# ariana-spalter/human-robot-gym

Hardware: AMD Instinct MI355X
Metric: env steps/sec (whole node), ReachHuman+shield 4096 envs (higher is better)
Workload: dtype f64

## Files before the change

human-robot-gym_amd/csrc/hrgym_device.h:

```cpp
#pragma once
#include <hip/hip_runtime.h>
#include <stdint.h>

#include "../../include/hrgym.h"
#include "../../include/hrgym_state.h"

#define NV HRG_NV
#define NARM HRG_NARM
#ifndef HRG_BOX
#define HRG_BOX 0
#endif
#ifndef HRG_LIFT
#define HRG_LIFT 0
#endif
#ifndef HRG_HANDOVER
#define HRG_HANDOVER 0
#endif
#ifndef HRG_STACK
#define HRG_STACK 0
#endif
#ifndef HRG_HULLS
#define HRG_HULLS 0
#endif
#ifndef HRG_HAMMER
// ... 126 lines not shown
  int32_t hb_maxdepth;
  double sol_K, sol_Bd;
  double rcap_hl[HRG_NRCAP], hcap_hl[HRG_NHB];
  int32_t hb_njump;
  int32_t hb_jump[4][HRG_NHB];
  int32_t phase_mask;
  hrg_path brake_full;
  double brake_T, brake_ds;
  int32_t hc_n;
  struct alignas(32) HcRec { double th, v, al; int32_t kj, pad; } hc[HRG_NHCAP_MAX];
  int32_t n_self;
  struct alignas(8) SelfPair { int32_t i, j; } self_ij[64];
  int32_t n_chk;
  int32_t chk_i[32], chk_j[32];
  hrg_clip_table clips;
  const double* pose_tab;
  const double* hull_dev;
  double hull_cen[HRG_NHULL][3];
  unsigned long long* mpr_fallback;
  double fric_D[NV + 1], fric_lim[NV + 1];
  double eul_hd[NV], eul_rhd[2];
  int32_t eul_fingers, eul_pad;
  double rcap_mid[HRG_NRCAP][3];
};

struct Contact {
  int32_t g1, g2, b1, b2;
  double dist, n[3], pos[3];
};

#define ROW_CON0 24
#define ROW_WELD0 (ROW_CON0 + 4 * NCON_DYN)
#if HRG_HAMMER
#define HROW_NFRIC 8
#define HROW_LIM0 9
#define HROW_NLIM 25
#define HROW_EQ0 27
#define HROW_CON0 36
#define HROW_NEQ 9
#define NROW 128
#elif HRG_STACK
#define SROW_WELD0 24
#define SROW_CON0 36
#define NROW HRG_NROW_STACK
#elif HRG_BOX && (HRG_HANDOVER || HRG_LIFT)
#define NROW (ROW_WELD0 + 6)
// ... 480 lines not shown
    if (g > 0) lo = w; else hi = w;
    const double sd = d1 >= 0 ? 1.0 : -1.0;
    const double T1p = sd * (fabs(d1) >= vtri ? 1.0 / amax : (fabs(d1) > 0 ? 1.0 / fsqrt(jmax * fabs(d1)) : 0.0));
    const double T2p = w >= vtri ? 1.0 / amax : (w > 0 ? 1.0 / fsqrt(jmax * w) : 0.0);
    const double dncp = 0.5 * T1 + 0.5 * (vm + w) * T1p + 0.5 * T2 + 0.5 * w * T2p;
    const double gp = T1p + T2p - dncp / w - rest / (w * w);
    double nw = gp < 0 ? w - g / gp : 0.5 * (lo + hi);
    if (!(nw > lo && nw < hi)) nw = 0.5 * (lo + hi);
    const double step = fabs(nw - w);
    w = nw;
    found = true;
    if (step <= 4e-16 * (1.0 + w) || hi - lo <= 4e-16 * (1.0 + hi)) break;
  }
  if (!found || !(w > 0)) return;
  const double tc = (Dm - dist_nocruise(vm, w, amax, jmax)) / w;
  if (!(tc >= 0)) return;
  int n = tl.n0;
  scurve(tl.v, tl.sg * w, amax, jmax, dur + n, jerk + n);
  n += 3;
  dur[n] = tc; jerk[n] = 0; n++;
  scurve(tl.sg * w, 0, amax, jmax, dur + n, jerk + n);
}

DI void ltt_eval(const hrg_ltt* L, int j, double s, double* q, double* v, double* a) {
  double qq = L->q0[j], vv = L->v0[j], aa = L->a0[j], t = s;
  if (t < 0) t = 0;
  for (int i = 0; i < HRG_LTT_NSEG; i++) {
    double d = L->dur[j][i], jj = L->jerk[j][i];
    if (t < d) {
      *q = qq + vv * t + 0.5 * aa * t * t + jj * t * t * t * SIXTH;
      *v = vv + aa * t + 0.5 * jj * t * t;
      *a = aa + jj * t;
      return;
    }
    qq += vv * d + 0.5 * aa * d * d + jj * d * d * d * SIXTH;
    vv += aa * d + 0.5 * jj * d * d;
    aa += jj * d;
    t -= d;
  }
  *q = L->qT[j]; *v = 0; *a = 0;
}

DI void ltt_eval2(const hrg_ltt* L, int j, double sa, double sb, double* qa, double* va, double* aa_, double* qb) {
  double qq = L->q0[j], vv = L->v0[j], aa = L->a0[j], ta = sa < 0 ? 0 : sa, tb = sb < 0 ? 0 : sb;
  bool done_a = false;
  for (int i = 0; i < HRG_LTT_NSEG; i++) {
    const double d = L->dur[j][i], jj = L->jerk[j][i];
    if (!done_a && ta < d) {
      *qa = qq + vv * ta + 0.5 * aa * ta * ta + jj * ta * ta * ta * SIXTH;
      *va = vv + aa * ta + 0.5 * jj * ta * ta;
      *aa_ = aa + jj * ta;
      done_a = true;
    }
    if (tb < d) {
      *qb = qq + vv * tb + 0.5 * aa * tb * tb + jj * tb * tb * tb * SIXTH;
      return;
    }
    qq += vv * d + 0.5 * aa * d * d + jj * d * d * d * SIXTH;
    vv += aa * d + 0.5 * jj * d * d;
    aa += jj * d;
    ta -= d;
    tb -= d;
  }
  if (!done_a) { *qa = L->qT[j]; *va = 0; *aa_ = 0; }
  *qb = L->qT[j];
}

__host__ DI void path_plan(hrg_path* P, double s0, double v0, double a0, double ve, double amax, double jmax) {
  P->s0 = s0; P->v0 = v0; P->a0 = a0; P->k = 0;
  for (int i = 0; i < 3; i++) { P->dur[i] = 0; P->jerk[i] = 0; }
  if (fabs(v0 - ve) < 1e-12 && fabs(a0) < 1e-12) { P->v0 = ve; P->a0 = 0; return; }
  double v_at = v0 + a0 * fabs(a0) / (2 * jmax);
  double dir = ve >= v_at ? 1.0 : -1.0;
  double A = dir * a0, dv = dir * (ve - v0);
  double apk = amax > A ? amax : A;
  double t1 = (apk - A) / jmax, t3 = apk / jmax;
  double dv2 = dv - 0.5 * (A + apk) * t1 - 0.5 * apk * t3, t2;
  if (dv2 >= 0) t2 = dv2 / apk;
  else {
    double r = 0.5 * A * A + jmax * dv;
    apk = sqrt(r > 0 ? r : 0);
    if (apk < A) apk = A;
    t1 = (apk - A) / jmax; t2 = 0; t3 = apk / jmax;
  }
  P->dur[0] = t1; P->dur[1] = t2; P->dur[2] = t3;
  P->jerk[0] = dir * jmax; P->jerk[1] = 0; P->jerk[2] = -dir * jmax;
}
__host__ DI double path_total(const hrg_path* P) { return P->dur[0] + P->dur[1] + P->dur[2]; }
// ... 220 lines not shown
```

human-robot-gym_amd/csrc/hrgym_hip.hip:

```cpp
#include <hip/hip_runtime.h>

#include <algorithm>
#include <cmath>
#include <cstdio>
#include <cstring>
#include <cstdlib>
#include <initializer_list>
#include <limits>
#include <memory>
#include <string>
#include <vector>

#include "hrgym_kernels.h"

template <class MD>
DI void impedance(const MD& m, double x0, double* imp) {
  const double d0 = m.solimp[0], dmax = m.solimp[1], width = m.solimp[2], mid = m.solimp[3], power = m.solimp[4];
  const double x = fabs(x0) / width;
  double y;
  if (x >= 1) y = 1;
  else if (x <= 0) y = 0;
  else if (x <= mid) { const double u = x / mid; y = u * u * mid; }
  else { const double u = (1 - x) / (1 - mid); y = 1 - u * u * (1 - mid); }
  (void)power;
// ... 2358 lines not shown
    eef_update(dm_);
    s.low_level_time = s.low_level_time + 1;
  }
  wave_sync();
  STAMP_FLUSH(lane);
  return crash | busy_out;
}

DI int env_step(const DevModel* __restrict__ dm_, int lane, int e, int64_t own_gid, double* __restrict__ action, float* obs, float* term_obs,
                 float* reward, uint8_t* done, int32_t* info, double* dbg_r, double* dbg_h, int32_t* dbg_nh, int32_t* fair) {
  const ModelPtr dm = uniform_model(dm_);
  Lds& L = g_L;
  const auto& m = dm->m;
  hrg_env_state& s = L.st;
  (void)fair;
  const int64_t gid = s.stream_id;
  int has_collision = 0, collision_type = HRG_COL_NULL, crash = 0;
  STAMP_INIT(lane);
  if (lane < NV) L.act[lane] = lane < HRG_ACT_DIM ? action[lane] : 0.0;
  wave_sync();
#if HRG_POSE_TABLE
  human_yaw_update();
#endif
  if (m.ik_enabled) ik_action(dm_, lane);
  if (m.cp_enabled) screen_action(dm_, lane, gid);
#if HRG_LIFT
  if (m.task == HRG_TASK_LIFTING) { wave_sync(); if (lane == 0) L.act[NARM] = 1.0; wave_sync(); }
#endif
#if HRG_HAMMER
  if (!m.gripper_controllable) { wave_sync(); if (lane == 0) L.act[NARM] = 1.0; wave_sync(); }
#endif
  if ((m.cp_enabled || m.ik_enabled) && lane < HRG_ACT_DIM) action[lane] = L.act[lane];
  s.timestep = s.timestep + 1;
  L.acc_has_collision = 0; L.acc_collision_type = HRG_COL_NULL; L.acc_failsafe = 0;
  wave_sync();
  int busy = 0;
#pragma unroll 1
  for (int cyc = 0; cyc < m.n_cycles && !crash; cyc++) { const int r = cycle_body(dm_, lane, e, gid, cyc, busy, dbg_r, dbg_h, dbg_nh, fair); crash = r & 1; busy = r >> 1; }
#if HRG_FAIR
  fair_publish(fair, lane, -1);
  __builtin_amdgcn_s_setprio(0);
#endif
  has_collision = L.acc_has_collision; collision_type = L.acc_collision_type;
  double goal[NARM];
  for (int j = 0; j < NARM; j++) goal[j] = s.cur_goal[j];
#if HRG_BOX
// ... 601 lines not shown
  }
  if (lane < NV) { st[HRG_MC_EUL_HD + lane] = dm_->eul_hd[lane]; re[HRG_MC_EUL_HD + lane] = c.eul_hd; }
  if (lane < 2) { st[HRG_MC_EUL_RHD + lane] = dm_->eul_rhd[lane]; re[HRG_MC_EUL_RHD + lane] = c.eul_rhd; }
  if (lane == 0) { st[HRG_MC_EUL_FINGERS] = dm_->eul_fingers; re[HRG_MC_EUL_FINGERS] = c.eul_fingers; }
  if (lane < 3 * HRG_NRCAP) { st[HRG_MC_RCAP_MID + lane] = (&dm_->rcap_mid[0][0])[lane]; re[HRG_MC_RCAP_MID + lane] = c.rcap_mid; }
}
#endif

__global__ __launch_bounds__(64) void HRG_SYM(hrg_chain_fk_kernel)(const DevModel* __restrict__ dm_, const double* __restrict__ q, int n, int shield_on, double* __restrict__ out) {
  const int lane = hrg_lane(), k = (int)blockIdx.x;
  if (k >= n) return;
  Lds& L = g_L;
  const double* qk = q + (size_t)k * 3 * NARM;
  if (lane < NARM) { L.cq[lane] = qk[lane]; L.qe[lane] = qk[NARM + lane]; }
  if (lane < NV) L.st.qpos[lane] = lane < NARM ? qk[2 * NARM + lane] : 0.0;
  wave_sync();
  robot_chain_fk(dm_, lane, shield_on != 0);
  double* o = out + (size_t)k * HRG_CFK_DIM;
  for (int j = lane; j < 9 * NV; j += 64) o[HRG_CFK_KR + j] = (&L.kR[0][0])[j];
  if (lane < 3 * NV) o[HRG_CFK_KP + lane] = (&L.kp[0][0])[lane];
  for (int j = lane; j < 2 * HRG_NSHIELD_RCAP * 6; j += 64) o[HRG_CFK_SCAP + j] = shield_on ? (&L.scap[0][0][0])[j] : 0.0;
}

#define HRG_NP_HAS_BOX (HRG_BOX || HRG_STACK || HRG_HAMMER)
#define HRG_NP_HAS_BB (HRG_STACK || HRG_HAMMER || HRG_LIFT)
#define HRG_NP_BOX_LANES 32
#define HRG_NP_BB_LANES (HRG_STACK ? 6 : HRG_HAMMER ? 4 : 1)
__global__ __launch_bounds__(64) void HRG_SYM(hrg_narrowphase_kernel)(int kind, const double* __restrict__ qs, int n, double* __restrict__ out) {
  const int lane = hrg_lane(), per = kind == HRG_NP_SEGSEG ? 64 : kind == HRG_NP_BOXBOX ? HRG_NP_BB_LANES : HRG_NP_BOX_LANES, k = (int)blockIdx.x * per + lane;
  const bool on = lane < per && k < n;
  const double* q = qs + (size_t)(on ? k : 0) * HRG_NP_QDIM;
  double* o = out + (size_t)(on ? k : 0) * HRG_NP_ODIM;
  if (on) for (int a = 0; a < HRG_NP_ODIM; a++) o[a] = 0.0;
  if (kind == HRG_NP_SEGSEG) {
    if (on) {
      double c1[3], c2[3];
      o[0] = seg_seg(q, q + 3, q + 6, q + 9, c1, c2);
      for (int a = 0; a < 3; a++) { o[1 + a] = c1[a]; o[4 + a] = c2[a]; }
    }
    return;
  }
#if HRG_NP_HAS_BOX || HRG_NP_HAS_BB
  Lds& L = g_L;
  double* W = &L.Jc[0][0];
  const int sl = on ? lane : 0;
#endif
// ... 53 lines not shown
    return;
  }
#endif
}

typedef void hrg_launch_step_fn(int n_envs, hipStream_t st, const DevModel* dm, hrg_env_state* states, double* actions, float* obs, float* term_obs, float* reward, uint8_t* done,
                                int32_t* info, double* dbg_r, double* dbg_h, int32_t* dbg_nh, int64_t env_id0, float* scratch_obs, void* objs, StepOrder ord);
typedef void hrg_launch_reset_fn(int n_envs, hipStream_t st, const DevModel* dm, hrg_env_state* states, const uint8_t* mask, float* obs, int64_t env_id0, void* objs);
extern "C" __attribute__((visibility("hidden"))) hrg_launch_step_fn HRG_SYM(hrg_launch_step);
extern "C" __attribute__((visibility("hidden"))) hrg_launch_reset_fn HRG_SYM(hrg_launch_reset);
extern "C" void HRG_SYM(hrg_launch_step)(int n_envs, hipStream_t st, const DevModel* dm, hrg_env_state* states, double* actions, float* obs, float* term_obs, float* reward, uint8_t* done,
                                         int32_t* info, double* dbg_r, double* dbg_h, int32_t* dbg_nh, int64_t env_id0, float* scratch_obs, void* objs, StepOrder ord) {
  hipLaunchKernelGGL(HRG_SYM(hrg_step_kernel), HRG_LAUNCH_DIMS(n_envs), 0, st, dm, states, actions, obs, term_obs, reward, done, info, dbg_r, dbg_h, dbg_nh, env_id0, scratch_obs, (ObjState*)objs,
                     n_envs, ord);
}
extern "C" void HRG_SYM(hrg_launch_reset)(int n_envs, hipStream_t st, const DevModel* dm, hrg_env_state* states, const uint8_t* mask, float* obs, int64_t env_id0, void* objs) {
  hipLaunchKernelGGL(HRG_SYM(hrg_reset_kernel), HRG_LAUNCH_DIMS(n_envs), 0, st, dm, states, mask, obs, env_id0, (ObjState*)objs, n_envs);
}
typedef void hrg_launch_chain_fk_fn(int n, const DevModel* dm, const double* q, int shield_on, double* out);
extern "C" __attribute__((visibility("hidden"))) hrg_launch_chain_fk_fn HRG_SYM(hrg_launch_chain_fk);
extern "C" void HRG_SYM(hrg_launch_chain_fk)(int n, const DevModel* dm, const double* q, int shield_on, double* out) {
  hipLaunchKernelGGL(HRG_SYM(hrg_chain_fk_kernel), dim3((unsigned)n), dim3(64), 0, 0, dm, q, n, shield_on, out);
}
typedef int hrg_launch_narrowphase_fn(int kind, int n, const double* q, double* out);
extern "C" __attribute__((visibility("hidden"))) hrg_launch_narrowphase_fn HRG_SYM(hrg_launch_narrowphase);
extern "C" int HRG_SYM(hrg_launch_narrowphase)(int kind, int n, const double* q, double* out) {
  const bool has = kind == HRG_NP_SEGSEG || (HRG_NP_HAS_BOX && (kind == HRG_NP_SEGBOX || kind == HRG_NP_CAPBOX)) || (HRG_NP_HAS_BB && kind == HRG_NP_BOXBOX);
  if (!has) return 0;
  const int per = kind == HRG_NP_SEGSEG ? 64 : kind == HRG_NP_BOXBOX ? HRG_NP_BB_LANES : HRG_NP_BOX_LANES;
  hipLaunchKernelGGL(HRG_SYM(hrg_narrowphase_kernel), dim3((unsigned)((n + per - 1) / per)), dim3(64), 0, 0, kind, q, n, out);
  return 1;
}

#ifdef HRG_STAMPS
#if HRG_BASE_TU
extern "C" int hrg_debug_stamps_slow(double* out, unsigned long long thresh, int reset) {
  unsigned long long h[34];
  if (hipMemcpyFromSymbol(h, HIP_SYMBOL(g_stamps_slow), sizeof h) != hipSuccess) return -1;
  for (int i = 0; i < 34; i++) out[i] = (double)h[i];
  if (reset) { memset(h, 0, sizeof h); hipMemcpyToSymbol(HIP_SYMBOL(g_stamps_slow), h, sizeof h); }
  hipMemcpyToSymbol(HIP_SYMBOL(g_slow_thresh), &thresh, sizeof thresh);
  return 0;
}
#endif
extern "C" int HRG_SYM(hrg_debug_stamps)(double* out, int reset) {
  unsigned long long h[32];
// ... 27 lines not shown
```

human-robot-gym_amd/csrc/hrgym_host_batch.h:

```cpp

struct TaskTraits;
struct hrg_batch {
  int device = 0;
  int32_t n_envs = 0;
  int64_t env_id0 = 0;
  DeviceMem mem;
  DevModel* d_model = nullptr;
  double* d_frames = nullptr;
  double* d_pose = nullptr;
  size_t pose_bytes = 0;
  double* d_hull = nullptr;
  bool hulls = false;
  unsigned long long* d_mpr_fallback = nullptr;
  hrg_env_state* d_states = nullptr;
  double* d_rcaps = nullptr;
  double* d_hcaps = nullptr;
  int32_t* d_nh = nullptr;
  float* d_scratch_obs = nullptr;
  hrg_box_state* d_boxes = nullptr;
  hrg_stack_state* d_stacks = nullptr;
  hrg_hammer_state* d_hammers = nullptr;
  int32_t* d_order = nullptr;
  int32_t parity = 0;
  const TaskTraits* traits = nullptr;
  bool ik = false;
  bool has_expert = false;
  hrg_expert_desc expert;
  ExpertBuffers ex;
  std::unique_ptr<DeviceMem> ex_mem;
  bool has_dataset = false;
  hrg_dataset_desc dataset;
  DatasetDev ds;
  std::unique_ptr<DeviceMem> ds_mem;
// ... 11 lines not shown
  static int32_t* tab[64] = {nullptr};
  if (device < 0 || device >= 64) return nullptr;
  if (!tab[device]) {
    int32_t* p = nullptr;
    if (hipMalloc(&p, sizeof(int32_t) * HRG_FAIR_SLOTS) != hipSuccess) return nullptr;
    if (hipMemset(p, 0, sizeof(int32_t) * HRG_FAIR_SLOTS) != hipSuccess) { hipFree(p); return nullptr; }
    tab[device] = p;
  }
  return tab[device];
}

enum { HRG_FAM_REACH, HRG_FAM_BOX, HRG_FAM_HO, HRG_FAM_LIFT, HRG_FAM_STACK, HRG_FAM_HAMMER, HRG_NFAMILY };
#define HRG_VARIANTS(X)                                              \
  X(HRG_FAM_REACH, 0, )          X(HRG_FAM_REACH, 1, _hull)          \
  X(HRG_FAM_BOX, 0, _box)        X(HRG_FAM_BOX, 1, _box_hull)        \
  X(HRG_FAM_HO, 0, _ho)          X(HRG_FAM_HO, 1, _ho_hull)          \
  X(HRG_FAM_LIFT, 0, _lift)      X(HRG_FAM_LIFT, 1, _lift_hull)      \
  X(HRG_FAM_STACK, 0, _stack)    X(HRG_FAM_STACK, 1, _stack_hull)    \
  X(HRG_FAM_HAMMER, 0, _hammer)  X(HRG_FAM_HAMMER, 1, _hammer_hull)
#define X(family, hulls, sfx)                                                                  \
  extern "C" __attribute__((visibility("hidden"))) hrg_launch_step_fn hrg_launch_step##sfx;    \
  extern "C" __attribute__((visibility("hidden"))) hrg_launch_reset_fn hrg_launch_reset##sfx;  \
  extern "C" __attribute__((visibility("hidden"))) hrg_launch_chain_fk_fn hrg_launch_chain_fk##sfx;  \
  extern "C" __attribute__((visibility("hidden"))) hrg_launch_narrowphase_fn hrg_launch_narrowphase##sfx;
HRG_VARIANTS(X)
#undef X
struct Variant { hrg_launch_step_fn* step; hrg_launch_reset_fn* reset; hrg_launch_chain_fk_fn* chain_fk; hrg_launch_narrowphase_fn* narrowphase; };
struct VariantTable { Variant v[HRG_NFAMILY][2]; };
static constexpr VariantTable make_variants() {
  VariantTable t{};
#define X(family, hulls, sfx) t.v[family][hulls] = Variant{hrg_launch_step##sfx, hrg_launch_reset##sfx, hrg_launch_chain_fk##sfx, hrg_launch_narrowphase##sfx};
  HRG_VARIANTS(X)
#undef X
  return t;
}
static const VariantTable g_variants = make_variants();

enum { HRG_OBJ_NONE, HRG_OBJ_BOXES, HRG_OBJ_STACKS, HRG_OBJ_HAMMERS };
struct TaskTraits {
  int task, family, objs;
  bool pose_table;
  bool dataset;
  unsigned experts, sirs;
};
#define E(x) (1u << HRG_EXPERT_##x)
#define S(x) (1u << HRG_SIR_##x)
static constexpr TaskTraits HRG_TASKS[] = {
  {HRG_TASK_REACH, HRG_FAM_REACH, HRG_OBJ_NONE, true, true, E(REACH), S(REACH)},
  {HRG_TASK_PICK_PLACE, HRG_FAM_BOX, HRG_OBJ_BOXES, false, true, E(PICK_PLACE), S(PICK_PLACE)},
  {HRG_TASK_INSPECTION, HRG_FAM_BOX, HRG_OBJ_BOXES, false, true, 0, 0},
  {HRG_TASK_POINTING, HRG_FAM_BOX, HRG_OBJ_BOXES, false, true, 0, 0},
  {HRG_TASK_HANDOVER_H2R, HRG_FAM_HO, HRG_OBJ_BOXES, false, true, E(PICK_PLACE), S(PICK_PLACE)},
  {HRG_TASK_HANDOVER_R2H, HRG_FAM_HO, HRG_OBJ_BOXES, false, true, E(PICK_PLACE), S(PICK_PLACE)},
  {HRG_TASK_LIFTING, HRG_FAM_LIFT, HRG_OBJ_BOXES, true, true, E(LIFTING), S(LIFTING)},
// ... 184 lines not shown
    double se, ve, ae;
    path_plan(&hm->brake_full, 0.0, 1.0, 0.0, desc->failsafe_sdot, desc->path_amax, desc->path_jmax);
    hm->brake_T = path_total(&hm->brake_full);
    path_eval(&hm->brake_full, hm->brake_T, desc->failsafe_sdot, &se, &ve, &ae);
    hm->brake_ds = se;
  }
#ifdef HRG_STAMPS
  if (const char* pm = getenv("HRG_PHASE_MASK")) hm->phase_mask = atoi(pm);
#endif
  hm->clips = *clips;
  if (desc->robot_hulls) hull_centroids(desc->hull_verts, desc->hull_off, hm->hull_cen);
}

static int batch_upload(hrg_batch* b, const hrg_model_desc* desc, const hrg_clip_table* clips, DevModel* hm) {
  DeviceMem& m = b->mem;
  const size_t frames = (size_t)clips->total_frames;
  bool ok = m.upload(b->d_frames, clips->frames, HRG_FRAME_DIM * frames);
  if (ok && b->traits->pose_table) {
    b->pose_bytes = sizeof(double) * HRG_POSE_DIM * frames;
    ok = m.zeros(b->d_pose, HRG_POSE_DIM * frames);
  }
  if (ok && desc->robot_hulls)
    ok = m.upload(b->d_hull, desc->hull_verts, 3 * (size_t)desc->hull_off[HRG_NHULL]) && m.zeros(b->d_mpr_fallback, 1);
  hm->clips.frames = b->d_frames;
  hm->pose_tab = b->d_pose;
  hm->hull_dev = b->d_hull;
  hm->mpr_fallback = b->d_mpr_fallback;
  if (!ok || !m.upload(b->d_model, hm, 1)) return nomem("batch", m);
  hipLaunchKernelGGL(hrg_model_constants_kernel, dim3(1), dim3(64), 0, 0, b->d_model);
  HIPCHK(hipGetLastError());
  HIPCHK(hipDeviceSynchronize());
  if (b->d_pose) {
    hipLaunchKernelGGL(hrg_pose_table_kernel, dim3((unsigned)clips->total_frames), dim3(64), 0, 0, b->d_model, b->d_pose);
    HIPCHK(hipGetLastError());
    HIPCHK(hipDeviceSynchronize());
  }
  return HRG_OK;
}

static int batch_env_arrays(hrg_batch* b) {
  const size_t n = (size_t)b->n_envs;
  std::vector<hrg_env_state> init(n);
  memset(init.data(), 0, sizeof(hrg_env_state) * n);
  for (auto& s : init) s.episode = -1;
  std::vector<int32_t> ord(2 * n + 4, 0);
  for (size_t e = 0; e < n; e++) ord[e] = ord[n + e] = (int32_t)e;
  DeviceMem& m = b->mem;
// ... 369 lines not shown
  }), "hrg_debug_cull_box");
}

int hrg_debug_model_constants(hrg_batch* b, double* out_host) {
  if (!b || !out_host) return fail(HRG_ERR_INVALID, "null argument");
  HIPCHK(hipSetDevice(b->device));
  return tap_result(hrg_run_tap(nullptr, 0, out_host, sizeof(double) * 2 * HRG_MC_DIM, [&](void** d) {
    hipMemset(d[0], 0, sizeof(double) * 2 * HRG_MC_DIM);
    hipLaunchKernelGGL(hrg_model_constants_tap_kernel, dim3(1), dim3(64), 0, 0, b->d_model, 0.0, (double*)d[0]);
  }), "hrg_debug_model_constants");
}

int hrg_debug_chain_fk(hrg_batch* b, const double* q_host, int32_t n, int32_t shield_on, double* out_host) {
  if (!b || !q_host || !out_host || n < 1 || n > 64) return fail(HRG_ERR_INVALID, "null argument or n outside 1..64");
  HIPCHK(hipSetDevice(b->device));
  void* objs;
  const Variant& v = batch_variant(b, &objs);
  const TapBuf in[] = {{q_host, sizeof(double) * 3 * NARM * (size_t)n}};
  return tap_result(hrg_run_tap(in, 1, out_host, sizeof(double) * HRG_CFK_DIM * (size_t)n, [&](void** d) {
    v.chain_fk((int)n, b->d_model, (const double*)d[0], shield_on ? 1 : 0, (double*)d[1]);
  }), "hrg_debug_chain_fk");
}

int hrg_debug_narrowphase(hrg_batch* b, int32_t kind, const double* queries_host, int32_t n, double* out_host) {
  if (!b || !queries_host || !out_host || n < 1 || n > HRG_NP_MAX) return fail(HRG_ERR_INVALID, "null argument or n outside 1..HRG_NP_MAX");
  if (kind < HRG_NP_SEGSEG || kind > HRG_NP_BOXBOX) return fail(HRG_ERR_INVALID, "no such kind of narrowphase query");
  HIPCHK(hipSetDevice(b->device));
  void* objs;
  const Variant& v = batch_variant(b, &objs);
  bool has = true;
  const TapBuf in[] = {{queries_host, sizeof(double) * HRG_NP_QDIM * (size_t)n}};
  const bool ok = hrg_run_tap(in, 1, out_host, sizeof(double) * HRG_NP_ODIM * (size_t)n, [&](void** d) {
    has = v.narrowphase((int)kind, (int)n, (const double*)d[0], (double*)d[1]) != 0;
  });
  if (!has) return fail(HRG_ERR_UNSUPPORTED, "this batch's kernel variant does not compile that routine");
  return tap_result(ok, "hrg_debug_narrowphase");
}

}
```

human-robot-gym_amd/csrc/hrgym_kernels.h:

```cpp
#pragma once
#include "hrgym_device.h"
#if HRG_HULLS
#include "hrgym_hull.h"
#endif

DI double chain_dot(double a0, double a1, double a2, double b0, double b1, double b2) {
#pragma clang fp contract(off)
  return __builtin_fma(a2, b2, __builtin_fma(a0, b0, a1 * b1));
}
DI double chain_acc(double a0, double a1, double a2, double b0, double b1, double b2) {
  return __builtin_fma(a2, b2, __builtin_fma(a1, b1, __builtin_fma(a0, b0, 0.0)));
}
DI void robot_chain_fk(const DevModel* __restrict__ dm_, int lane, bool shield_on) {
  const ModelPtr dm = uniform_model(dm_);
  Lds& L = g_L;
  if (lane < 3 * NARM && (lane >= 2 * NARM || shield_on)) {
    const int cfg = lane / NARM, i = lane - NARM * cfg;
    const double q = cfg == 0 ? L.cq[i] : (cfg == 1 ? L.qe[i] : L.st.qpos[i]);
    double sn, cs;
    sincos_small(q, &sn, &cs);
    LdsF64* o = lds_lane_base(&L.rc[0][0] + 2 * lane);
    o[0] = sn; o[1] = cs;
  }
  wave_sync();
// ... 496 lines not shown
    clip = clip_of(dm, gid, s.episode, anim_index);
  }
  s.anim_index = anim_index; s.anim_start_time = anim_start; s.animation_time = at;
#if HRG_BOX
  human_pose_fk(dm_, lane, clip, at, hold_body, hold_left);
#else
  human_pose_fk(dm_, lane, clip, at);
#endif
}

PH_SHIELD void shield_step(const DevModel* __restrict__ dm_, int lane, int e, double* __restrict__ dbg_r, double* __restrict__ dbg_h, int32_t* __restrict__ dbg_nh) {
  const ModelPtr dm = uniform_model(dm_);
  Lds& L = g_L;
  const auto& m = dm->m;
  hrg_env_state& s = L.st;
  const double dt = m.timestep, t = s.time;
  const bool shield_on = m.shield_type != HRG_SHIELD_OFF;
  const bool have_vel = s.n_meas >= 1 && t > s.meas_prev_t;
  if (lane < NARM) { L.cq[lane] = s.des_q[lane]; L.cv[lane] = s.des_v[lane]; L.ca[lane] = s.des_a[lane]; }
  wave_sync();
  int use_cand = 0;
  if (s.new_goal) {
    double nq = 0, nv = 0, na = 0;
    if (lane < NARM) ltt_eval(&s.ltt, lane, s.path_s, &nq, &nv, &na);
    const bool bad = lane < NARM && fabs(na) > m.a_max_ltt[lane];
    if (!__any(bad)) {
      use_cand = 1;
      double tj = 0;
      LttTail tail;
      tail.n0 = 0; tail.v = tail.sg = tail.Dm = tail.vm = tail.w = 0;
      if (lane < NARM) {
        ltt_plan_joint(&L.cand, lane, nq, nv, na, s.new_goal_q[lane], m.v_max_ltt[lane], m.a_max_ltt[lane], m.j_max_ltt[lane], &tail);
        for (int i = 0; i < HRG_LTT_NSEG; i++) tj += L.cand.dur[lane][i];
      }
      const double Tall = wave_max(tj);
      L.cand.T = Tall;
      if (m.ltt_time_sync && lane < NARM) ltt_sync_joint(&L.cand, lane, Tall, m.a_max_ltt[lane], m.j_max_ltt[lane], tail);
    }
    wave_sync();
  }
  STAMP(10);
  const hrg_ltt* Lp = use_cand ? &L.cand : &s.ltt;
  const double ps = use_cand ? 0.0 : s.path_s, pv = s.path_v, pa = s.path_a;
  hrg_path fs2;
  double s1, v1, a1, se, Tb;
  const bool pfl = m.shield_type == HRG_SHIELD_PFL, steady = pv == 1.0 && pa == 0.0;
  if (steady) { s1 = ps + dt; v1 = 1.0; a1 = 0.0; }
  else {
    hrg_path rec;
    path_plan(&rec, ps, pv, pa, 1.0, m.path_amax, m.path_jmax);
    path_eval(&rec, dt, 1.0, &s1, &v1, &a1);
  }
  double ve_fs = m.failsafe_sdot;
  if (pfl) {
    double q_, d1_ = 0, d2_;
    if (lane < NARM) ltt_eval(Lp, lane, s1, &q_, &d1_, &d2_);
    const double vc = wave_sum(lane < NARM ? fabs(d1_) * m.pfl_reach[lane] : 0.0);
    ve_fs = vc > m.pfl_v_safe ? m.pfl_v_safe / vc : 1.0;
  }
  if (steady && !pfl) {
    fs2.s0 = s1; fs2.v0 = 1.0; fs2.a0 = 0.0; fs2.k = 0.0;
    for (int a = 0; a < 3; a++) { fs2.dur[a] = dm->brake_full.dur[a]; fs2.jerk[a] = dm->brake_full.jerk[a]; }
    Tb = dm->brake_T;
    se = s1 + dm->brake_ds;
  } else {
    double ve_, ae;
    path_plan(&fs2, s1, v1, a1, ve_fs, m.path_amax, m.path_jmax);
    Tb = path_total(&fs2);
    path_eval(&fs2, Tb, ve_fs, &se, &ve_, &ae);
  }
  s1 = uniform_f64(s1); v1 = uniform_f64(v1); a1 = uniform_f64(a1); se = uniform_f64(se); Tb = uniform_f64(Tb);
  fs2.s0 = uniform_f64(fs2.s0); fs2.v0 = uniform_f64(fs2.v0); fs2.a0 = uniform_f64(fs2.a0); fs2.k = uniform_f64(fs2.k);
  for (int a = 0; a < 3; a++) { fs2.dur[a] = uniform_f64(fs2.dur[a]); fs2.jerk[a] = uniform_f64(fs2.jerk[a]); }
  STAMP(11);
  if (shield_on && lane < NARM) {
    double qn, q1, q2, qv;
    ltt_eval2(Lp, lane, s1, se, &qn, &q1, &q2, &qv);
    L.qe[lane] = qv;
    s.des_q[lane] = qn; s.des_v[lane] = q1 * v1; s.des_a[lane] = q1 * a1 + q2 * v1 * v1;
  }
  wave_sync();
  STAMP(12);
  robot_chain_fk(dm_, lane, shield_on);
  STAMP(13);
  int safe = 1;
  if (shield_on) {
    const double sdiff = se - ps;
    double rc_hl = 0;
    if (lane < HRG_NSHIELD_RCAP) {
      const int c = lane;
      double d[3], l1, l2;
      v3sub(d, &L.scap[0][c][0], &L.scap[1][c][0]); l1 = v3norm(d);
      v3sub(d, &L.scap[0][c][3], &L.scap[1][c][3]); l2 = v3norm(d);
      for (int a = 0; a < 6; a++) L.rc[c][a] = 0.5 * (L.scap[0][c][a] + L.scap[1][c][a]);
      L.rc[c][6] = m.scap_r[c] + m.secure_radius + 0.5 * (l1 > l2 ? l1 : l2) + m.scap_alpha[c] * sdiff * sdiff / 8.0;
      double hv[3];
      for (int a = 0; a < 3; a++) hv[a] = 0.5 * (L.rc[c][3 + a] - L.rc[c][a]);
      rc_hl = fsqrt(v3dot(hv, hv));
      L.scap[0][c][0] = rc_hl;
      if (dbg_r) for (int a = 0; a < 7; a++) dbg_r[((size_t)e * HRG_NSHIELD_RCAP + c) * 7 + a] = L.rc[c][a];
// ... 67 lines not shown
            const double reach = L.scap[0][c][0] + hl + rr + 1e-9;
            close = !(v3dot(dc, dc) > reach * reach);
          }
          if (!__any(close)) continue;
          if (close) { double x1[3], x2[3]; if (seg_seg(&L.rc[c][0], &L.rc[c][3], c1, c2, x1, x2) < rr * rr) hit = true; }
          if (__any(hit)) break;
        }
      }
      all_hit = __any(hit);
    }
    safe = !all_hit;
  }
  wave_sync();
  STAMP(14);
  for (int k = lane; k < HRG_NHJ * 3; k += 64) (&s.meas_prev[0][0])[k] = (&s.human_site[0][0])[k];
  s.meas_prev_t = t;
  if (s.n_meas < 2) s.n_meas = s.n_meas + 1;
  if (safe) {
    if (use_cand) {
      double* dst = (double*)&s.ltt;
      const double* src = (const double*)&L.cand;
      for (int k = lane; k < (int)(sizeof(hrg_ltt) / sizeof(double)); k += 64) dst[k] = src[k];
      s.new_goal = 0;
    }
    s.path_s = s1; s.path_v = v1; s.path_a = a1;
    s.safe_path = fs2;
  } else {
    const double k = s.safe_path.k + 1.0;
    s.safe_path.k = k;
    double ns, nv, na;
    const hrg_path spc = s.safe_path;
    const double vend = pfl ? path_vend(&spc) : m.failsafe_sdot;
    path_eval(&s.safe_path, k * dt, vend, &ns, &nv, &na);
    if (use_cand && s.path_v <= vend + 1e-9 && fabs(s.path_a) <= 1e-9) {
      const double adv = ns - s.path_s;
      double* dst = (double*)&s.ltt;
      const double* src = (const double*)&L.cand;
      for (int q = lane; q < (int)(sizeof(hrg_ltt) / sizeof(double)); q += 64) dst[q] = src[q];
      s.new_goal = 0;
      ns = adv;
      hrg_path sp;
      path_plan(&sp, ns, nv, na, vend, m.path_amax, m.path_jmax);
      s.safe_path = sp;
    }
    s.path_s = ns; s.path_v = nv; s.path_a = na;
  }
  s.is_safe = safe;
  wave_sync();
  if (lane < NARM && !(shield_on && safe)) {
    double qq, q1, q2;
    ltt_eval(&s.ltt, lane, s.path_s, &qq, &q1, &q2);
    s.des_q[lane] = qq; s.des_v[lane] = q1 * s.path_v; s.des_a[lane] = q1 * s.path_a + q2 * s.path_v * s.path_v;
  }
  wave_sync();
  STAMP(15);
}

DI void shield_reset(const DevModel* __restrict__ , int lane) {
  Lds& L = g_L;
  hrg_env_state& s = L.st;
  if (lane < NARM) {
    const double q = s.qpos[lane];
    s.ltt.q0[lane] = q; s.ltt.qT[lane] = q;
    s.des_q[lane] = q; s.new_goal_q[lane] = q; s.goal_qpos[lane] = q;
  }
  s.is_safe = 1;
}

#if HRG_STACK || HRG_HAMMER || HRG_LIFT
#define BB_TIE 1e-9
#define BB_ON (1 + 1e-12)
struct BBContact { double pos[3], n[3], dist; };
#define BB_WORK 152
DI int box_box2(const double* pa, const double* Ra, const double* ha, const double* pb, const double* Rb, const double* hb, BBContact* out, double* T) {
// ... 924 lines not shown
```

include/hrgym.h:

```cpp
#ifndef HRGYM_H
#define HRGYM_H

#include <stddef.h>
#include <stdint.h>

#ifdef __cplusplus
extern "C" {
#endif

#define HRG_NARM 6
#define HRG_NFINGER 2
#define HRG_NV (HRG_NARM + HRG_NFINGER)
#define HRG_NHB 24
#define HRG_NHJ 23
#define HRG_NHQ 69
#define HRG_NRCAP 10
#define HRG_NHULL 7
#define HRG_NSHIELD_RCAP 7
#define HRG_NBODYPART_MAX 20
#define HRG_NEXTREMITY_MAX 4
#define HRG_NHCAP_MAX 64
#define HRG_LTT_NSEG 12
#define HRG_OBS_DIM 64
#define HRG_ACT_DIM 7
// ... 469 lines not shown
int hrg_batch_get_box(hrg_batch* b, int32_t env, void* buf_host, size_t bytes);
int hrg_batch_set_box(hrg_batch* b, int32_t env, const void* buf_host, size_t bytes);
size_t hrg_stack_bytes(void);
int hrg_batch_get_stack(hrg_batch* b, int32_t env, void* buf_host, size_t bytes);
int hrg_batch_set_stack(hrg_batch* b, int32_t env, const void* buf_host, size_t bytes);
size_t hrg_hammer_bytes(void);
int hrg_batch_get_hammer(hrg_batch* b, int32_t env, void* buf_host, size_t bytes);
int hrg_batch_set_hammer(hrg_batch* b, int32_t env, const void* buf_host, size_t bytes);
int hrg_test_hull_queries(const double* verts_host, const int32_t* off_host, const void* queries_host, int32_t n, double* out_host);
int hrg_test_hull_box_queries(const double* verts_host, const int32_t* off_host, const void* queries_host, int32_t n, double* out_host);
int hrg_batch_mpr_fallbacks(hrg_batch* b, int64_t* count_host);
int hrg_batch_pose_table_bytes(hrg_batch* b, int64_t* bytes_host);
int hrg_debug_pose_compare(hrg_batch* b, const void* queries_host, int32_t n, double* out_host);
enum { HRG_WAVE_NOUT = 22  };
int hrg_debug_wave_helpers(const double* in_host, uint64_t lane_mask, double* out_host);
int hrg_debug_cull_box(const double* in_host, int32_t n, double* out_host);
enum { HRG_MC_FRIC_D = 0, HRG_MC_FRIC_LIM = HRG_NV + 1, HRG_MC_FRIC_IMP = 2 * (HRG_NV + 1), HRG_MC_EUL_HD = 3 * (HRG_NV + 1), HRG_MC_EUL_RHD = HRG_MC_EUL_HD + HRG_NV,
       HRG_MC_EUL_FINGERS = HRG_MC_EUL_RHD + 2, HRG_MC_RCAP_MID = HRG_MC_EUL_FINGERS + 1, HRG_MC_DIM = HRG_MC_RCAP_MID + 3 * HRG_NRCAP };
int hrg_debug_model_constants(hrg_batch* b, double* out_host);
enum { HRG_CFK_KR = 0, HRG_CFK_KP = 9 * HRG_NV, HRG_CFK_SCAP = 12 * HRG_NV, HRG_CFK_DIM = HRG_CFK_SCAP + 2 * HRG_NSHIELD_RCAP * 6 };
int hrg_debug_chain_fk(hrg_batch* b, const double* q_host, int32_t n, int32_t shield_on, double* out_host);
enum { HRG_NP_SEGSEG = 0, HRG_NP_SEGBOX = 1, HRG_NP_CAPBOX = 2, HRG_NP_BOXBOX = 3, HRG_NP_QDIM = 24, HRG_NP_ODIM = 32, HRG_NP_MAX = 4096 };
int hrg_debug_narrowphase(hrg_batch* b, int32_t kind, const double* queries_host, int32_t n, double* out_host);

int hrg_batch_check_actions(hrg_batch* b, const double* actions_dev, uint8_t* collides_dev, void* hip_stream);

int hrg_batch_expert_attach(hrg_batch* b, const hrg_expert_desc* desc);
int hrg_batch_expert_actions(hrg_batch* b, const float* obs_dev, double* actions_out_dev, void* stream);
int hrg_batch_step_imitation(hrg_batch* b, double* actions_dev, float* obs_dev, float* term_obs_dev, float* reward_dev, uint8_t* done_dev, int32_t* info_dev,
                             float* imit_dev, void* stream);

int hrg_batch_snapshot(hrg_batch* b, void* states_out_dev, void* boxes_out_dev, void* stream);
int hrg_batch_dataset_attach(hrg_batch* b, const hrg_dataset_desc* desc);
int hrg_batch_dataset_reset(hrg_batch* b, const uint8_t* mask_dev, float* obs_dev, void* stream);
int hrg_batch_step_dataset(hrg_batch* b, double* actions_dev, float* obs_dev, float* term_obs_dev, float* reward_dev, uint8_t* done_dev, int32_t* info_dev,
                           float* imit_dev, float* sir_dev, void* stream);
int hrg_batch_dataset_cursor(hrg_batch* b, int32_t* cursor_host);

int hrg_her_create(const hrg_her_desc* desc, int32_t device, hrg_her** out);
void hrg_her_destroy(hrg_her* h);
int hrg_her_observe(hrg_her* h, const float* obs_dev, const uint8_t* mask_dev, int64_t* counts_dev, void* stream);
int hrg_her_add(hrg_her* h, const double* actions_dev, const float* obs_dev, const float* term_obs_dev, const float* reward_dev, const uint8_t* done_dev,
                const int32_t* info_dev, int64_t* counts_dev, void* stream);
int hrg_her_sample(hrg_her* h, int32_t batch_size, const int64_t* counts_cum_dev, float* observation_dev, float* achieved_goal_dev, float* desired_goal_dev,
                   float* next_observation_dev, float* next_achieved_goal_dev, float* next_desired_goal_dev, float* action_dev, float* reward_dev,
                   float* done_dev, int64_t* index_dev, void* stream);
// ... 94 lines not shown
```

Baseline: 4.945 million.

## Precompute per-segment trajectory knots in global memory for faster LTT evaluation

Adds a per-env global buffer holding the position, velocity and acceleration at the start of each trajectory segment, filled at the start of every env step and again whenever a new trajectory is adopted. Evaluations then find the segment and do a single cubic evaluation instead of advancing through every earlier segment. The polynomial arithmetic is rewritten with explicit FMAs so knot-based and direct evaluation give identical results, and a debug kernel compares the two. The cost is extra global writes and reads on every step, including a full knot rebuild each step even when the trajectory has not changed.

After: 4.975 million, median of 6. Within noise of the previous version (+0.6%).

```diff
diff --git a/human-robot-gym_amd/csrc/hrgym_device.h b/human-robot-gym_amd/csrc/hrgym_device.h
--- a/human-robot-gym_amd/csrc/hrgym_device.h
+++ b/human-robot-gym_amd/csrc/hrgym_device.h
@@ -172,6 +172,7 @@
   double eul_hd[NV], eul_rhd[2];
   int32_t eul_fingers, eul_pad;
   double rcap_mid[HRG_NRCAP][3];
+  double* ltt_knots;
 };
 
 struct Contact {
@@ -698,20 +699,40 @@
   scurve(tl.sg * w, 0, amax, jmax, dur + n, jerk + n);
 }
 
+DI double ltt_cubic_q(double qq, double vv, double aa, double jj, double t) {
+#pragma clang fp contract(off)
+  double r = __builtin_fma(t, vv, qq), u = t * jj;
+  r = __builtin_fma(t, (0.5 * aa) * t, r);
+  u = t * u; u = t * u;
+  return __builtin_fma(SIXTH, u, r);
+}
+DI double ltt_cubic_v(double vv, double aa, double jj, double t) {
+#pragma clang fp contract(off)
+  return __builtin_fma(t, t * (0.5 * jj), __builtin_fma(aa, t, vv));
+}
+DI void ltt_advance(double& qq, double& vv, double& aa, double jj, double d) {
+#pragma clang fp contract(off)
+  double t = (0.5 * aa) * d, u = d * jj, w = 0.5 * jj;
+  t = d * t; t = __builtin_fma(vv, d, t);
+  u = d * u; u = d * u; t = __builtin_fma(SIXTH, u, t);
+  w = d * w; w = d * w; w = __builtin_fma(aa, d, w);
+  qq = qq + t;
+  vv = vv + w;
+  aa = __builtin_fma(d, jj, aa);
+}
+
 DI void ltt_eval(const hrg_ltt* L, int j, double s, double* q, double* v, double* a) {
   double qq = L->q0[j], vv = L->v0[j], aa = L->a0[j], t = s;
   if (t < 0) t = 0;
   for (int i = 0; i < HRG_LTT_NSEG; i++) {
     double d = L->dur[j][i], jj = L->jerk[j][i];
     if (t < d) {
-      *q = qq + vv * t + 0.5 * aa * t * t + jj * t * t * t * SIXTH;
-      *v = vv + aa * t + 0.5 * jj * t * t;
-      *a = aa + jj * t;
+      *q = ltt_cubic_q(qq, vv, aa, jj, t);
+      *v = ltt_cubic_v(vv, aa, jj, t);
+      *a = __builtin_fma(t, jj, aa);
       return;
     }
-    qq += vv * d + 0.5 * aa * d * d + jj * d * d * d * SIXTH;
-    vv += aa * d + 0.5 * jj * d * d;
-    aa += jj * d;
+    ltt_advance(qq, vv, aa, jj, d);
     t -= d;
   }
   *q = L->qT[j]; *v = 0; *a = 0;
@@ -723,23 +744,76 @@
   for (int i = 0; i < HRG_LTT_NSEG; i++) {
     const double d = L->dur[j][i], jj = L->jerk[j][i];
     if (!done_a && ta < d) {
-      *qa = qq + vv * ta + 0.5 * aa * ta * ta + jj * ta * ta * ta * SIXTH;
-      *va = vv + aa * ta + 0.5 * jj * ta * ta;
-      *aa_ = aa + jj * ta;
+      *qa = ltt_cubic_q(qq, vv, aa, jj, ta);
+      *va = ltt_cubic_v(vv, aa, jj, ta);
+      *aa_ = __builtin_fma(ta, jj, aa);
       done_a = true;
     }
     if (tb < d) {
-      *qb = qq + vv * tb + 0.5 * aa * tb * tb + jj * tb * tb * tb * SIXTH;
+      *qb = ltt_cubic_q(qq, vv, aa, jj, tb);
       return;
     }
-    qq += vv * d + 0.5 * aa * d * d + jj * d * d * d * SIXTH;
-    vv += aa * d + 0.5 * jj * d * d;
-    aa += jj * d;
+    ltt_advance(qq, vv, aa, jj, d);
     ta -= d;
     tb -= d;
   }
   if (!done_a) { *qa = L->qT[j]; *va = 0; *aa_ = 0; }
   *qb = L->qT[j];
+}
+
+#define HRG_KNOT_DIM 3
+#define HRG_KNOT_ROW (NARM * HRG_LTT_NSEG * HRG_KNOT_DIM)
+typedef double __attribute__((address_space(1)))* KnotPtr;
+DI KnotPtr ltt_knot_row(ModelPtr dm, int e, int j) { return (KnotPtr)dm->ltt_knots + (size_t)e * HRG_KNOT_ROW + j * (HRG_LTT_NSEG * HRG_KNOT_DIM); }
+DI void ltt_knots(const hrg_ltt* L, int j, KnotPtr K) {
+  double qq = L->q0[j], vv = L->v0[j], aa = L->a0[j];
+#pragma unroll 1
+  for (int i = 0; i < HRG_LTT_NSEG; i++) {
+    K[HRG_KNOT_DIM * i] = qq; K[HRG_KNOT_DIM * i + 1] = vv; K[HRG_KNOT_DIM * i + 2] = aa;
+    if (i == HRG_LTT_NSEG - 1) break;
+    ltt_advance(qq, vv, aa, L->jerk[j][i], L->dur[j][i]);
+  }
+}
+DI int ltt_find(const hrg_ltt* L, int j, double s, double* tl) {
+  double t = s < 0 ? 0 : s;
+  int hit = -1;
+#pragma unroll 1
+  for (int i = 0; i < HRG_LTT_NSEG; i++) {
+    const double d = L->dur[j][i];
+    if (t < d) { hit = i; break; }
+    t -= d;
+  }
+  *tl = t;
+  return hit;
+}
+DI void ltt_eval_k(const hrg_ltt* L, const KnotPtr K, int j, double s, double* q, double* v, double* a) {
+  double t;
+  const int i = ltt_find(L, j, s, &t);
+  if (i < 0) { *q = L->qT[j]; *v = 0; *a = 0; return; }
+  const double qq = K[HRG_KNOT_DIM * i], vv = K[HRG_KNOT_DIM * i + 1], aa = K[HRG_KNOT_DIM * i + 2], jj = L->jerk[j][i];
+  *q = ltt_cubic_q(qq, vv, aa, jj, t);
+  *v = ltt_cubic_v(vv, aa, jj, t);
+  *a = __builtin_fma(t, jj, aa);
+}
+DI void ltt_eval2_k(const hrg_ltt* L, const KnotPtr K, int j, double sa, double sb, double* qa, double* va, double* aa_, double* qb) {
+  double ta = sa < 0 ? 0 : sa, tb = sb < 0 ? 0 : sb;
+  int ia = -1, ib = -1;
+#pragma unroll
+  for (int i = 0; i < HRG_LTT_NSEG; i++) {
+    const double d = L->dur[j][i];
+    if (ia < 0) { if (ta < d) ia = i; else ta -= d; }
+    if (tb < d) { ib = i; break; }
+    tb -= d;
+  }
+  if (ia < 0) { *qa = L->qT[j]; *va = 0; *aa_ = 0; }
+  else {
+    const double qq = K[HRG_KNOT_DIM * ia], vv = K[HRG_KNOT_DIM * ia + 1], aa = K[HRG_KNOT_DIM * ia + 2], jj = L->jerk[j][ia];
+    *qa = ltt_cubic_q(qq, vv, aa, jj, ta);
+    *va = ltt_cubic_v(vv, aa, jj, ta);
+    *aa_ = __builtin_fma(ta, jj, aa);
+  }
+  if (ib < 0) *qb = L->qT[j];
+  else *qb = ltt_cubic_q(K[HRG_KNOT_DIM * ib], K[HRG_KNOT_DIM * ib + 1], K[HRG_KNOT_DIM * ib + 2], L->jerk[j][ib], tb);
 }
 
 __host__ DI void path_plan(hrg_path* P, double s0, double v0, double a0, double ve, double amax, double jmax) {
diff --git a/human-robot-gym_amd/csrc/hrgym_hip.hip b/human-robot-gym_amd/csrc/hrgym_hip.hip
--- a/human-robot-gym_amd/csrc/hrgym_hip.hip
+++ b/human-robot-gym_amd/csrc/hrgym_hip.hip
@@ -2404,6 +2404,7 @@
 #if HRG_POSE_TABLE
   human_yaw_update();
 #endif
+  if (lane < NARM) ltt_knots(&s.ltt, lane, ltt_knot_row(dm, e, lane));
   if (m.ik_enabled) ik_action(dm_, lane);
   if (m.cp_enabled) screen_action(dm_, lane, gid);
 #if HRG_LIFT
@@ -3051,6 +3052,33 @@
   for (int j = lane; j < 2 * HRG_NSHIELD_RCAP * 6; j += 64) o[HRG_CFK_SCAP + j] = shield_on ? (&L.scap[0][0][0])[j] : 0.0;
 }
 
+__global__ __launch_bounds__(64) void HRG_SYM(hrg_ltt_eval_kernel)(const DevModel* __restrict__ dm_, const double* __restrict__ q, int n, double* __restrict__ out) {
+  const ModelPtr dm = uniform_model(dm_);
+  const int lane = hrg_lane(), k = (int)blockIdx.x;
+  if (k >= n) return;
+  hrg_env_state& s = g_L.st;
+  const double* qk = q + (size_t)k * HRG_LTTQ_DIM;
+  constexpr int NL = (int)(sizeof(hrg_ltt) / sizeof(double));
+  static_assert(NL + 2 == HRG_LTTQ_DIM, "a query is an hrg_ltt and two path positions");
+  for (int i = lane; i < NL; i += 64) ((double*)&s.ltt)[i] = qk[i];
+  wave_sync();
+  if (lane >= NARM) return;
+  const double sa = qk[NL], sb = qk[NL + 1];
+  double* o = out + (size_t)k * HRG_LTTO_DIM + 4 * lane;
+  double dv, da;
+  ltt_eval2(&s.ltt, lane, sa, sb, o, o + 1, o + 2, o + 3);
+  const KnotPtr K = ltt_knot_row(dm, k, lane);
+  ltt_knots(&s.ltt, lane, K);
+  o += 4 * NARM;
+  ltt_eval2_k(&s.ltt, K, lane, sa, sb, o, o + 1, o + 2, o + 3);
+  o += 4 * NARM;
+  ltt_eval(&s.ltt, lane, sa, o, o + 1, o + 2);
+  ltt_eval(&s.ltt, lane, sb, o + 3, &dv, &da);
+  o += 4 * NARM;
+  ltt_eval_k(&s.ltt, K, lane, sa, o, o + 1, o + 2);
+  ltt_eval_k(&s.ltt, K, lane, sb, o + 3, &dv, &da);
+}
+
 #define HRG_NP_HAS_BOX (HRG_BOX || HRG_STACK || HRG_HAMMER)
 #define HRG_NP_HAS_BB (HRG_STACK || HRG_HAMMER || HRG_LIFT)
 #define HRG_NP_BOX_LANES 32
@@ -3150,6 +3178,11 @@
 extern "C" void HRG_SYM(hrg_launch_chain_fk)(int n, const DevModel* dm, const double* q, int shield_on, double* out) {
   hipLaunchKernelGGL(HRG_SYM(hrg_chain_fk_kernel), dim3((unsigned)n), dim3(64), 0, 0, dm, q, n, shield_on, out);
 }
+typedef void hrg_launch_ltt_eval_fn(int n, const DevModel* dm, const double* q, double* out);
+extern "C" __attribute__((visibility("hidden"))) hrg_launch_ltt_eval_fn HRG_SYM(hrg_launch_ltt_eval);
+extern "C" void HRG_SYM(hrg_launch_ltt_eval)(int n, const DevModel* dm, const double* q, double* out) {
+  hipLaunchKernelGGL(HRG_SYM(hrg_ltt_eval_kernel), dim3((unsigned)n), dim3(64), 0, 0, dm, q, n, out);
+}
 typedef int hrg_launch_narrowphase_fn(int kind, int n, const double* q, double* out);
 extern "C" __attribute__((visibility("hidden"))) hrg_launch_narrowphase_fn HRG_SYM(hrg_launch_narrowphase);
 extern "C" int HRG_SYM(hrg_launch_narrowphase)(int kind, int n, const double* q, double* out) {
diff --git a/human-robot-gym_amd/csrc/hrgym_host_batch.h b/human-robot-gym_amd/csrc/hrgym_host_batch.h
--- a/human-robot-gym_amd/csrc/hrgym_host_batch.h
+++ b/human-robot-gym_amd/csrc/hrgym_host_batch.h
@@ -9,6 +9,7 @@
   double* d_frames = nullptr;
   double* d_pose = nullptr;
   size_t pose_bytes = 0;
+  double* d_knots = nullptr;
   double* d_hull = nullptr;
   bool hulls = false;
   unsigned long long* d_mpr_fallback = nullptr;
@@ -66,14 +67,15 @@
   extern "C" __attribute__((visibility("hidden"))) hrg_launch_step_fn hrg_launch_step##sfx;    \
   extern "C" __attribute__((visibility("hidden"))) hrg_launch_reset_fn hrg_launch_reset##sfx;  \
   extern "C" __attribute__((visibility("hidden"))) hrg_launch_chain_fk_fn hrg_launch_chain_fk##sfx;  \
-  extern "C" __attribute__((visibility("hidden"))) hrg_launch_narrowphase_fn hrg_launch_narrowphase##sfx;
+  extern "C" __attribute__((visibility("hidden"))) hrg_launch_narrowphase_fn hrg_launch_narrowphase##sfx;  \
+  extern "C" __attribute__((visibility("hidden"))) hrg_launch_ltt_eval_fn hrg_launch_ltt_eval##sfx;
 HRG_VARIANTS(X)
 #undef X
-struct Variant { hrg_launch_step_fn* step; hrg_launch_reset_fn* reset; hrg_launch_chain_fk_fn* chain_fk; hrg_launch_narrowphase_fn* narrowphase; };
+struct Variant { hrg_launch_step_fn* step; hrg_launch_reset_fn* reset; hrg_launch_chain_fk_fn* chain_fk; hrg_launch_narrowphase_fn* narrowphase; hrg_launch_ltt_eval_fn* ltt_eval; };
 struct VariantTable { Variant v[HRG_NFAMILY][2]; };
 static constexpr VariantTable make_variants() {
   VariantTable t{};
-#define X(family, hulls, sfx) t.v[family][hulls] = Variant{hrg_launch_step##sfx, hrg_launch_reset##sfx, hrg_launch_chain_fk##sfx, hrg_launch_narrowphase##sfx};
+#define X(family, hulls, sfx) t.v[family][hulls] = Variant{hrg_launch_step##sfx, hrg_launch_reset##sfx, hrg_launch_chain_fk##sfx, hrg_launch_narrowphase##sfx, hrg_launch_ltt_eval##sfx};
   HRG_VARIANTS(X)
 #undef X
   return t;
@@ -304,7 +306,9 @@
   }
   if (ok && desc->robot_hulls)
     ok = m.upload(b->d_hull, desc->hull_verts, 3 * (size_t)desc->hull_off[HRG_NHULL]) && m.zeros(b->d_mpr_fallback, 1);
+  ok = ok && m.zeros(b->d_knots, (size_t)HRG_KNOT_ROW * (size_t)b->n_envs);
   hm->clips.frames = b->d_frames;
+  hm->ltt_knots = b->d_knots;
   hm->pose_tab = b->d_pose;
   hm->hull_dev = b->d_hull;
   hm->mpr_fallback = b->d_mpr_fallback;
@@ -720,6 +724,17 @@
   }), "hrg_debug_chain_fk");
 }
 
+int hrg_debug_ltt_eval(hrg_batch* b, const double* queries_host, int32_t n, double* out_host) {
+  if (!b || !queries_host || !out_host || n < 1 || n > 64 || n > b->n_envs) return fail(HRG_ERR_INVALID, "null argument or n outside 1..min(64, n_envs)");
+  HIPCHK(hipSetDevice(b->device));
+  void* objs;
+  const Variant& v = batch_variant(b, &objs);
+  const TapBuf in[] = {{queries_host, sizeof(double) * HRG_LTTQ_DIM * (size_t)n}};
+  return tap_result(hrg_run_tap(in, 1, out_host, sizeof(double) * HRG_LTTO_DIM * (size_t)n, [&](void** d) {
+    v.ltt_eval((int)n, b->d_model, (const double*)d[0], (double*)d[1]);
+  }), "hrg_debug_ltt_eval");
+}
+
 int hrg_debug_narrowphase(hrg_batch* b, int32_t kind, const double* queries_host, int32_t n, double* out_host) {
   if (!b || !queries_host || !out_host || n < 1 || n > HRG_NP_MAX) return fail(HRG_ERR_INVALID, "null argument or n outside 1..HRG_NP_MAX");
   if (kind < HRG_NP_SEGSEG || kind > HRG_NP_BOXBOX) return fail(HRG_ERR_INVALID, "no such kind of narrowphase query");
diff --git a/human-robot-gym_amd/csrc/hrgym_kernels.h b/human-robot-gym_amd/csrc/hrgym_kernels.h
--- a/human-robot-gym_amd/csrc/hrgym_kernels.h
+++ b/human-robot-gym_amd/csrc/hrgym_kernels.h
@@ -542,7 +542,9 @@
   int use_cand = 0;
   if (s.new_goal) {
     double nq = 0, nv = 0, na = 0;
-    if (lane < NARM) ltt_eval(&s.ltt, lane, s.path_s, &nq, &nv, &na);
+    if (lane < NARM) {
+      ltt_eval_k(&s.ltt, ltt_knot_row(dm, e, lane), lane, s.path_s, &nq, &nv, &na);
+    }
     const bool bad = lane < NARM && fabs(na) > m.a_max_ltt[lane];
     if (!__any(bad)) {
       use_cand = 1;
@@ -574,7 +576,10 @@
   double ve_fs = m.failsafe_sdot;
   if (pfl) {
     double q_, d1_ = 0, d2_;
-    if (lane < NARM) ltt_eval(Lp, lane, s1, &q_, &d1_, &d2_);
+    if (lane < NARM) {
+      if (!use_cand) ltt_eval_k(&s.ltt, ltt_knot_row(dm, e, lane), lane, s1, &q_, &d1_, &d2_);
+      else ltt_eval(Lp, lane, s1, &q_, &d1_, &d2_);
+    }
     const double vc = wave_sum(lane < NARM ? fabs(d1_) * m.pfl_reach[lane] : 0.0);
     ve_fs = vc > m.pfl_v_safe ? m.pfl_v_safe / vc : 1.0;
   }
@@ -595,7 +600,8 @@
   STAMP(11);
   if (shield_on && lane < NARM) {
     double qn, q1, q2, qv;
-    ltt_eval2(Lp, lane, s1, se, &qn, &q1, &q2, &qv);
+    if (!use_cand) ltt_eval2_k(&s.ltt, ltt_knot_row(dm, e, lane), lane, s1, se, &qn, &q1, &q2, &qv);
+    else ltt_eval2(Lp, lane, s1, se, &qn, &q1, &q2, &qv);
     L.qe[lane] = qv;
     s.des_q[lane] = qn; s.des_v[lane] = q1 * v1; s.des_a[lane] = q1 * a1 + q2 * v1 * v1;
   }
@@ -709,6 +715,7 @@
       const double* src = (const double*)&L.cand;
       for (int k = lane; k < (int)(sizeof(hrg_ltt) / sizeof(double)); k += 64) dst[k] = src[k];
       s.new_goal = 0;
+      if (lane < NARM) ltt_knots(&L.cand, lane, ltt_knot_row(dm, e, lane));
     }
     s.path_s = s1; s.path_v = v1; s.path_a = a1;
     s.safe_path = fs2;
@@ -725,6 +732,7 @@
       const double* src = (const double*)&L.cand;
       for (int q = lane; q < (int)(sizeof(hrg_ltt) / sizeof(double)); q += 64) dst[q] = src[q];
       s.new_goal = 0;
+      if (lane < NARM) ltt_knots(&L.cand, lane, ltt_knot_row(dm, e, lane));
       ns = adv;
       hrg_path sp;
       path_plan(&sp, ns, nv, na, vend, m.path_amax, m.path_jmax);
@@ -736,7 +744,7 @@
   wave_sync();
   if (lane < NARM && !(shield_on && safe)) {
     double qq, q1, q2;
-    ltt_eval(&s.ltt, lane, s.path_s, &qq, &q1, &q2);
+    ltt_eval_k(&s.ltt, ltt_knot_row(dm, e, lane), lane, s.path_s, &qq, &q1, &q2);
     s.des_q[lane] = qq; s.des_v[lane] = q1 * s.path_v; s.des_a[lane] = q1 * s.path_a + q2 * s.path_v * s.path_v;
   }
   wave_sync();
diff --git a/include/hrgym.h b/include/hrgym.h
--- a/include/hrgym.h
+++ b/include/hrgym.h
@@ -515,6 +515,8 @@
 int hrg_debug_chain_fk(hrg_batch* b, const double* q_host, int32_t n, int32_t shield_on, double* out_host);
 enum { HRG_NP_SEGSEG = 0, HRG_NP_SEGBOX = 1, HRG_NP_CAPBOX = 2, HRG_NP_BOXBOX = 3, HRG_NP_QDIM = 24, HRG_NP_ODIM = 32, HRG_NP_MAX = 4096 };
 int hrg_debug_narrowphase(hrg_batch* b, int32_t kind, const double* queries_host, int32_t n, double* out_host);
+enum { HRG_LTTQ_DIM = (4 + 2 * HRG_LTT_NSEG) * HRG_NARM + 3, HRG_LTTO_DIM = 4 * HRG_NARM * 4 };
+int hrg_debug_ltt_eval(hrg_batch* b, const double* queries_host, int32_t n, double* out_host);
 
 int hrg_batch_check_actions(hrg_batch* b, const double* actions_dev, uint8_t* collides_dev, void* hip_stream);
 
```
